# taichi-dev/voxel-rt2

Hardware: AMD Instinct MI355X
Metric: Mpath-samples/sec at 1920x1080, 8 bounces (higher is better)
Workload: dtype f32; 1 GPU; example1-style scene S1 (scenes.scene_s1), 128^3 grid, 1920x1080, 4 spp/step, 8 bounces, static camera, ReSTIR off; width=1920, height=1080, max_depth=8, seed=0, build_id=fbd5f3073040a2f2

## Files before the change

voxel_rt2_amd/csrc/vrt_kernels.hip:

```cpp
#include <hip/hip_runtime.h>
#include <cstdlib>
#include <atomic>
#include "vrt_kernels.h"
#include "vrt_probe.h"
#include "vrt_shade_probe.h"

namespace vrt {

template <int G>
__global__ void k_pack_grid(const int8_t* __restrict__ mat, const uint8_t* __restrict__ rgb, uint32_t* __restrict__ grid) {
    int i = blockIdx.x * blockDim.x + threadIdx.x;
    if (i >= G * G * G) return;
    int m = mat[i];
    uint32_t a = (m < 0) ? 0u : (uint32_t)m;
    const int z = i & (G - 1), y = (i / G) & (G - 1), x = i / (G * G);
    grid[texel_index<G>(x, y, z)] = (uint32_t)rgb[3 * i] | ((uint32_t)rgb[3 * i + 1] << 8) | ((uint32_t)rgb[3 * i + 2] << 16) | (a << 24);
}
__global__ void k_build_l0(const int8_t* __restrict__ mat, unsigned long long* __restrict__ l0, int G) {
    int b = blockIdx.x * blockDim.x + threadIdx.x;
    const int n0 = G >> 2;
    if (b >= n0 * n0 * n0) return;
    int bx = b % n0, by = (b / n0) % n0, bz = b / (n0 * n0);
    unsigned long long w = 0ULL;
    for (int z = 0; z < 4; z++)
// ... 355 lines not shown
    TraceStats ts;
    stats_zero(ts);
    bool exhausted = false;
    const unsigned tiles_per_range = ((unsigned)(tiles_x * tiles_y) + VRT_WORK_HEADS - 1u) / VRT_WORK_HEADS;
    const unsigned range = tiles_per_range * 64u * (unsigned)n_samples;
    const uint32_t prim_tag = drain_value;
    unsigned head = blockIdx.x & (VRT_WORK_HEADS - 1u);
    int heads_left = VRT_WORK_HEADS;
    unsigned q_cont = 0u, q_left = 0u;
    if constexpr (QUEUED) {
        q_cont = pq.counts[head * VRT_PV_COUNT_STRIDE]; q_left = pq.counts[head * VRT_PV_COUNT_STRIDE + 1];
        q_cont = q_cont < pq.cap ? q_cont : pq.cap; q_left = q_left < pq.left_cap ? q_left : pq.left_cap;
    }

#if defined(VRT_DIAG_REGIONS)
    unsigned long long t_prev = __builtin_readcyclecounter();
    int prev_stage = 4;
    unsigned long long t_stage[6] = {0ULL, 0ULL, 0ULL, 0ULL, 0ULL, 0ULL};
    unsigned long long t_sub[4] = {0ULL, 0ULL, 0ULL, 0ULL};
#define VRT_SUB_CLOCK(q) do { __asm__ volatile("s_waitcnt vmcnt(0) lgkmcnt(0)" ::: "memory"); const unsigned long long t_ = __builtin_readcyclecounter(); t_sub[q] += t_ - t_sub_prev; t_sub_prev = t_; } while (0)
#define VRT_SUB_START() do { __asm__ volatile("s_waitcnt vmcnt(0) lgkmcnt(0)" ::: "memory"); t_sub_prev = __builtin_readcyclecounter(); } while (0)
    unsigned long long t_sub_prev = 0ULL;
#define VRT_POOL_CLOCK(next_stage)                                                                              \
    do {                                                                                                        \
        const unsigned long long t_now = __builtin_readcyclecounter();                                          \
        _Pragma("unroll") for (int q_ = 0; q_ < 6; q_++) if (prev_stage == q_) t_stage[q_] += t_now - t_prev;   \
        t_prev = t_now; prev_stage = (next_stage);                                                              \
    } while (0)
#else
#define VRT_POOL_CLOCK(next_stage) ((void)0)
#define VRT_SUB_CLOCK(q) ((void)0)
#define VRT_SUB_START() ((void)0)
#endif
    for (;;) {
        wave_lds_sync();
        VRT_POOL_CLOCK(5);
        uint32_t st[WORDS];
        int cnt[4] = {0, 0, 0, 0};
#pragma unroll
        for (int k = 0; k < WORDS; k++) {
            st[k] = state[k * 64 + lane];
#pragma unroll
            for (int q = 0; q < 4; q++) cnt[q] += __popcll(__ballot(st[k] == (uint32_t)q));
        }
        if (exhausted) cnt[SLOT_EMPTY] = 0;
        int stage = SLOT_SHADE, best = cnt[SLOT_SHADE];
        if (cnt[SLOT_ESCAPE] > best) { stage = SLOT_ESCAPE; best = cnt[SLOT_ESCAPE]; }
        if (cnt[SLOT_RAY] > best) { stage = SLOT_RAY; best = cnt[SLOT_RAY]; }
        if (cnt[SLOT_EMPTY] > best) { stage = SLOT_EMPTY; best = cnt[SLOT_EMPTY]; }
        if (best == 0) break;
        int n = 0;
#pragma unroll
        for (int k = 0; k < WORDS; k++) {
            const bool mine = st[k] == (uint32_t)stage;
            const unsigned long long m = __ballot(mine);
            if (mine) list[n + lane_rank(m)] = (uint32_t)(k * 64 + lane);
            n += __popcll(m);
        }
        wave_lds_sync();
        VRT_POOL_CLOCK(stage);

        if (stage == SLOT_RAY) {
            VRT_REGION(14);
#ifndef VRT_POOL_PARK_MIN
#define VRT_POOL_PARK_MIN 64
#endif
            const int park = (n >= VRT_POOL_PARK_MIN) ? VRT_POOL_PARK : 0;
            int head = 0;
            bool active = false, ended = false;
            RayWalk w;
            BrickCache bc;
            bc.key = -1; bc.word = 0ULL;
            CoarseWords cw;
            cw.w1 = 0ULL; cw.w2 = 0ULL;
            SlotRef s;
            s.base = pool; s.stride = SLOTS;
            int slot = 0, iters0 = 0;
            for (;;) {
                const unsigned long long idle = __ballot(!active);
                const int n_idle = __popcll(idle);
                if (ended) {
                    VRT_REGION(16);
                    walk_store(s, w);
                    state[slot] = (uint32_t)slot_state_after_walk<G>(w.t, s.f(PF_FLOOR_T));
                    if (prim_cache) {
                        const uint32_t ids = s.u(PF_IDS);
                        if ((ids >> 24) == 0u)
                            primary_record_store(&prim_cache[((int)((ids >> 12) & 0xfffu) - fp.row0) * fp.W + (int)(ids & 0xfffu)], primary_record(s, prim_tag));
                    }
                    ts.iters += (unsigned)(w.iters - iters0);
                    ended = false;
                }
                if (head >= n) {
                    if (64 - n_idle <= park) {
                        if (active) {
                            VRT_REGION(17);
                            walk_store(s, w);
                            ts.iters += (unsigned)(w.iters - iters0);
                        }
                        break;
                    }
                } else {
                    const int idx = head + lane_rank(idle);
                    if (!active && idx < n) {
                        VRT_REGION(15);
                        slot = (int)list[idx];
                        s.base = pool + slot;
                        walk_load<G>(s, w);
                        coarse_fetch(P, w.ix, w.iy, w.iz, cw);
                        bc.key = -1;
                        iters0 = w.iters;
                        active = true;
                    }
                    head += (n_idle < n - head) ? n_idle : n - head;
                }
                const int target = (head < n) ? VRT_POOL_REFILL : 64 - park;
                do {
                    if (active) {
                        int nq;
                        if (walk_trip(P, w, bc, cw, nq)) { active = false; ended = true; }
                        ts.queries += (unsigned)nq;
                    }
                } while (__popcll(__ballot(!active)) < target);
            }
        } else {
            const int take = n < 64 ? n : 64;
            unsigned base = 0u, limit = 0u;
            unsigned range0 = 0u, per_sample = 1u;
            unsigned q_head = 0u, q_n_cont = 0u;
            if constexpr (QUEUED) {
              if (stage == SLOT_EMPTY) {
                VRT_SUB_START();
                unsigned got = 0u;
                if (lane == 0) got = atomicAdd(work_counter + head * VRT_WORK_HEAD_STRIDE, (unsigned)take);
                got = (unsigned)__builtin_amdgcn_readfirstlane((int)got);
                const unsigned cnt = q_cont + q_left;
                q_head = head; q_n_cont = q_cont;
                base = got;
                limit = (got + (unsigned)take < cnt) ? got + (unsigned)take : cnt;
                if (got + (unsigned)take >= cnt) {
                    heads_left -= 1;
                    head = (head + 1u) & (VRT_WORK_HEADS - 1u);
                    q_cont = pq.counts[head * VRT_PV_COUNT_STRIDE]; q_left = pq.counts[head * VRT_PV_COUNT_STRIDE + 1];
                    q_cont = q_cont < pq.cap ? q_cont : pq.cap; q_left = q_left < pq.left_cap ? q_left : pq.left_cap;
                    if (heads_left == 0) {
                        exhausted = true;
                        if (drain_signal && lane == 0 && atomicExch(work_counter + 1, 1u) == 0u)
                            __hip_atomic_fetch_max(drain_signal, drain_value, __ATOMIC_RELAXED, __HIP_MEMORY_SCOPE_SYSTEM);
                    }
                }
                if (base > limit) base = limit;
                VRT_SUB_CLOCK(0);
              }
            } else
            if (stage == SLOT_EMPTY) {
                VRT_SUB_START();
                unsigned got = 0u;
                if (lane == 0) got = atomicAdd(work_counter + head * VRT_WORK_HEAD_STRIDE, (unsigned)take);
                got = (unsigned)__builtin_amdgcn_readfirstlane((int)got);
                const unsigned r0 = head * range, r1 = (r0 + range < total) ? r0 + range : total;
                base = r0 + got;
                limit = (base + (unsigned)take < r1) ? base + (unsigned)take : r1;
                range0 = r0;
                per_sample = (r1 > r0) ? (r1 - r0) / (unsigned)n_samples : 1u;
                if (r0 >= total || base + (unsigned)take >= r1) {
                    heads_left -= 1;
                    head = (head + 1u) & (VRT_WORK_HEADS - 1u);
                    if (heads_left == 0) {
                        exhausted = true;
                        if (drain_signal && lane == 0 && atomicExch(work_counter + 1, 1u) == 0u)
                            __hip_atomic_fetch_max(drain_signal, drain_value, __ATOMIC_RELAXED, __HIP_MEMORY_SCOPE_SYSTEM);
                    }
                }
                if (base > limit) base = limit;
                VRT_SUB_CLOCK(0);
            }
            if (lane < take) {
                SlotRef s;
                s.stride = SLOTS;
                if (stage == SLOT_SHADE) {
                    VRT_REGION(11);
                    const int slot = (int)list[lane];
                    s.base = pool + slot;
                    state[slot] = (uint32_t)pool_shade<HIT_SOMETHING, BLACK_SUN, RESTIR>(fp, scl, P, out, s, cold_wave + slot * COLD, ts);
                } else if (stage == SLOT_ESCAPE) {
                    VRT_REGION(12);
                    const int slot = (int)list[lane];
                    s.base = pool + slot;
                    state[slot] = (uint32_t)pool_shade<HIT_NOTHING, false, RESTIR>(fp, scl, P, out, s, cold_wave + slot * COLD, ts);
                } else {
                    VRT_REGION(13);
                    const unsigned my = base + (unsigned)lane;
                    if constexpr (QUEUED) {
                        if (my < limit) {
                            const int slot = (int)list[lane];
                            s.base = pool + slot;
                            if (my < q_n_cont) {
                                constexpr int PW = PrimaryContWords<BLACK_SUN>::count;
                                const uint32_t* const at = pq.entries + ((size_t)q_head * pq.cap + my) * PW;
                                uint32_t e[PW];
#pragma unroll
                                for (int k = 0; k < PW; k++) e[k] = at[k];
                                VRT_SUB_CLOCK(1);
                                state[slot] = (uint32_t)pool_begin_queued<G, CULL, BLACK_SUN>(fp, scl.cull, s, cold_wave + slot * COLD, e, ts);
                                VRT_SUB_CLOCK(3);
                            } else {
                                const uint32_t item = pq.leftovers[(size_t)q_head * pq.left_cap + (my - q_n_cont)];
                                const int u = (int)(item & 0xfffu), v = (int)((item >> 12) & 0xfffu), sample = (int)(item >> 28);
                                const PrimaryRecord rec = primary_record_load(&prim_cache[(v - fp.row0) * fp.W + u]);
                                const bool known = primary_record_valid(rec, prim_tag);
                                VRT_SUB_CLOCK(1);
                                int st;
                                if (known) st = pool_begin_known<G>(fp, s, u, v, sample, rec);
                                else {
                                    st = pool_begin<G, CULL>(fp, scl.cull, s, u, v, sample, ts);
                                    if (sample == 0 && st != SLOT_RAY) primary_record_store(&prim_cache[(v - fp.row0) * fp.W + u], primary_record(s, prim_tag));
                                }
                                state[slot] = (uint32_t)st;
                                VRT_SUB_CLOCK(known ? 2 : 3);
                            }
                        }
                    } else
                    if (my < limit) {
                        const int slot = (int)list[lane];
                        s.base = pool + slot;
                        const unsigned j = my - range0;
                        const int sample = (int)(j >= per_sample) + (int)(j >= 2u * per_sample) + (int)(j >= 3u * per_sample);
                        const unsigned rem = j - (unsigned)sample * per_sample;
                        const unsigned tile = range0 / (64u * (unsigned)n_samples) + (rem >> 6), in = rem & 63u;
                        const int u = (int)(tile % (unsigned)tiles_x) * 8 + (int)(in & 7u);
                        const int v = launch_tile_row(fp, (int)(tile / (unsigned)tiles_x)) + (int)(in >> 3);
                        if (u < fp.W && v < fp.row1 && launch_renders_row(fp, v) && !outside_render_area(fp, (float)u, (float)v)) {
                            bool known = false;
                            PrimaryRecord rec;
                            rec.x = rec.y = rec.z = rec.dx = rec.dy = rec.dz = rec.ft = rec.w = 0u;
                            if (prim_cache && (SERVED || sample > 0)) {
                                rec = primary_record_load(&prim_cache[(v - fp.row0) * fp.W + u]);
                                known = primary_record_valid(rec, prim_tag);
                            }
                            VRT_SUB_CLOCK(1);
                            int st;
                            if (known) st = pool_begin_known<G>(fp, s, u, v, sample, rec);
                            else {
                                st = pool_begin<G, CULL>(fp, scl.cull, s, u, v, sample, ts);
                                if (prim_cache && sample == 0 && st != SLOT_RAY) primary_record_store(&prim_cache[(v - fp.row0) * fp.W + u], primary_record(s, prim_tag));
                            }
                            state[slot] = (uint32_t)st;
                            VRT_SUB_CLOCK(known ? 2 : 3);
                        }
                    }
                }
            }
        }
    }
    VRT_POOL_CLOCK(4);
#if defined(VRT_DIAG_REGIONS)
    if (lane == 0)
        for (int q = 0; q < 6; q++) atomicAdd(&g_vrt_region[2 * (20 + q)], t_stage[q]);
    if (lane == 0)
        for (int q = 0; q < 4; q++) atomicAdd(&g_vrt_region[52 + q], t_sub[q]);
#endif
    if (INSTR) flush_stats(ts, sc.counters);
}
template <int G, bool INSTR, bool BLACK_SUN, bool CULL, bool SERVED = false>
__global__ __launch_bounds__(64 * pool_shape<G>(false).waves, VRT_POOL_MIN_WAVES) __attribute__((amdgpu_num_vgpr(VRT_POOL_HALF_VGPRS))) void k_render_pool(FrameParams fp, SceneData sc, PixelBuffers out, unsigned* work_counter, unsigned* next_counter, int n_samples, uint32_t* cold, uint32_t* drain_signal, uint32_t drain_value, PrimaryRecord* prim_cache) {
    render_pool_body<G, false, INSTR, BLACK_SUN, CULL, false, SERVED>(fp, sc, out, work_counter, next_counter, n_samples, cold, drain_signal, drain_value, prim_cache);
}
template <int G, bool INSTR, bool CULL>
__global__ __launch_bounds__(64 * pool_shape<G>(true).waves, 3) __attribute__((amdgpu_num_vgpr(84))) void k_render_pool_dense12(FrameParams fp, SceneData sc, PixelBuffers out, unsigned* work_counter, unsigned* next_counter, int n_samples, uint32_t* cold, uint32_t* drain_signal, uint32_t drain_value, PrimaryRecord* prim_cache) {
    render_pool_body<G, false, INSTR, false, CULL, true>(fp, sc, out, work_counter, next_counter, n_samples, cold, drain_signal, drain_value, prim_cache);
}
template <int G, bool INSTR, bool CULL>
__global__ __launch_bounds__(64 * pool_shape<G>(false).waves, VRT_POOL_MIN_WAVES) __attribute__((amdgpu_num_vgpr(128))) void k_render_pool_restir(FrameParams fp, SceneData sc, PixelBuffers out, unsigned* work_counter, unsigned* next_counter, int n_samples, uint32_t* cold, uint32_t* drain_signal, uint32_t drain_value, PrimaryRecord* prim_cache) {
    render_pool_body<G, true, INSTR, false, CULL>(fp, sc, out, work_counter, next_counter, n_samples, cold, drain_signal, drain_value, prim_cache);
}

#ifndef VRT_PRIMARY_HALF_VGPRS
#define VRT_PRIMARY_HALF_VGPRS 48
#endif
template <int G, bool CULL>
__global__ __launch_bounds__(64) __attribute__((amdgpu_num_vgpr(VRT_PRIMARY_HALF_VGPRS))) void k_primary_records(FrameParams fp, SceneData sc, PrimaryRecord* prim_cache, uint32_t tag) {
    const int tiles_x = (fp.W + 7) >> 3;
    const unsigned tile = blockIdx.x, in = threadIdx.x;
    const int u = (int)(tile % (unsigned)tiles_x) * 8 + (int)(in & 7u);
    const int v = launch_tile_row(fp, (int)(tile / (unsigned)tiles_x)) + (int)(in >> 3);
    if (!(u < fp.W && v < fp.row1 && launch_renders_row(fp, v) && !outside_render_area(fp, (float)u, (float)v))) return;
    GlobalPyramid<G> P;
    P.p = sc.pyr;
    primary_record_store(&prim_cache[(v - fp.row0) * fp.W + u], primary_record_walk<G, CULL>(fp, P, sc.cull, u, v, tag));
}

#ifndef VRT_PRIMARY_VERTEX_HALF_VGPRS
#define VRT_PRIMARY_VERTEX_HALF_VGPRS 72
#endif
#ifndef VRT_PRIMARY_VERTEX_SUN_HALF_VGPRS
#define VRT_PRIMARY_VERTEX_SUN_HALF_VGPRS 84
#endif
#if 2 * VRT_PRIMARY_VERTEX_HALF_VGPRS + 2 * VRT_POOL_HALF_VGPRS > 512 || 2 * VRT_PRIMARY_VERTEX_SUN_HALF_VGPRS + 2 * VRT_POOL_HALF_VGPRS > 512
#error "k_primary_vertex must fit beside one pooled wave of a SIMD at least"
#endif
#ifndef VRT_PRIMARY_SHARED_SURF
#define VRT_PRIMARY_SHARED_SURF 1
#endif
template <int G, bool BLACK_SUN, bool CULL>
static __device__ __forceinline__ void primary_vertex_body(const FrameParams& fp, const SceneData& sc, const PixelBuffers& out, const PrimaryRecord* prim_cache, uint32_t tag, int n_samples, const PrimaryQueue& pq) {
    const int tiles_x = (fp.W + 7) >> 3;
    const unsigned tile = blockIdx.x, in = threadIdx.x;
    const int u = (int)(tile % (unsigned)tiles_x) * 8 + (int)(in & 7u);
    const int v = launch_tile_row(fp, (int)(tile / (unsigned)tiles_x)) + (int)(in >> 3);
    const bool live = u < fp.W && v < fp.row1 && launch_renders_row(fp, v) && !outside_render_area(fp, (float)u, (float)v);
    const unsigned head = tile & (VRT_PV_HEADS - 1u);
    constexpr int PW = PrimaryContWords<BLACK_SUN>::count;
    GlobalPyramid<G> P;
    P.p = sc.pyr;
    TraceStats ts;
    stats_zero(ts);
    PrimaryRecord rec;
    rec.x = rec.y = rec.z = rec.dx = rec.dy = rec.dz = rec.ft = rec.w = 0u;
    bool known = false;
    Hit h;
    hit_init(h);
    int state = SLOT_ESCAPE;
    constexpr bool SHARED_SURF = VRT_PRIMARY_SHARED_SURF != 0;
    Surf surf;
#if defined(VRT_DIAG_REGIONS)
    __shared__ unsigned long long pv_clock[PVR_COUNT + 1];
    if (in <= (unsigned)PVR_COUNT) pv_clock[in] = 0ULL;
    ts.pv = pv_clock;
    ts.pv[PVR_COUNT] = __builtin_readcyclecounter();
#endif
    if (live) {
        rec = primary_record_load(&prim_cache[(v - fp.row0) * fp.W + u]);
        known = primary_record_valid(rec, tag);
    }
    VRT_PV_CLOCK(ts, PVR_RECORD);
    if (known) {
        state = primary_vertex_hit<G>(fp, sc, rec, h, ts);
        primary_vertex_gbuffer(fp, out, u, v, rec, h);
        VRT_PV_CLOCK(ts, PVR_HIT);
        if constexpr (SHARED_SURF) (void)primary_vertex_surf<GlobalPyramid<G>>(sc, rec, h, state, surf);
        VRT_PV_CLOCK(ts, PVR_SURF);
    }
    unsigned n_done = 0u, n_on = 0u;
    for (int sample = 0; sample < n_samples; sample++) {
        Path<false> p;
        bool on = false;
        if (known) on = primary_vertex_sample<G, BLACK_SUN, CULL, SHARED_SURF>(fp, sc, P, out, u, v, sample, rec, h, state, p, ts, &surf);
        const unsigned long long m_on = __ballot(on);
        bool left = live && !known;
        if (m_on != 0ULL) {
            unsigned at = 0u;
            if (in == (unsigned)__builtin_ctzll(m_on)) at = atomicAdd(&pq.counts[head * VRT_PV_COUNT_STRIDE], (unsigned)__popcll(m_on));
            at = (unsigned)__shfl((int)at, __builtin_ctzll(m_on), 64) + (unsigned)__popcll(m_on & ((1ULL << in) - 1ULL));
            if (on) {
                if (at < pq.cap) primary_cont_pack<BLACK_SUN>(pq.entries + ((size_t)head * pq.cap + at) * PW, p);
                else left = true;
            }
        }
        const unsigned long long m_left = __ballot(left);
        if (m_left != 0ULL) {
            unsigned at = 0u;
            if (in == (unsigned)__builtin_ctzll(m_left)) at = atomicAdd(&pq.counts[head * VRT_PV_COUNT_STRIDE + 1], (unsigned)__popcll(m_left));
            at = (unsigned)__shfl((int)at, __builtin_ctzll(m_left), 64) + (unsigned)__popcll(m_left & ((1ULL << in) - 1ULL));
            if (left && at < pq.left_cap) pq.leftovers[(size_t)head * pq.left_cap + at] = primary_leftover_item(u, v, sample);
        }
        if (known && !left) { if (on) n_on++; else n_done++; }
        VRT_PV_CLOCK(ts, PVR_APPEND);
    }
#if defined(VRT_DIAG_REGIONS)
    if (in < (unsigned)PVR_COUNT) atomicAdd(&g_vrt_region[56 + in], pv_clock[in]);
    static_assert(56 + PVR_COUNT <= 64, "the region counters' last eight words");
#endif
    if (pq.report) {
        unsigned long long a = n_done, b = n_on;
        for (int off = 32; off > 0; off >>= 1) { a += __shfl_down(a, off, 64); b += __shfl_down(b, off, 64); }
        if (in == 0u) { atomicAdd(&pq.report[0], a); atomicAdd(&pq.report[1], b); }
    }
}
template <int G, bool CULL>
__global__ __launch_bounds__(64) __attribute__((amdgpu_num_vgpr(VRT_PRIMARY_VERTEX_HALF_VGPRS))) void k_primary_vertex(FrameParams fp, SceneData sc, PixelBuffers out, const PrimaryRecord* prim_cache, uint32_t tag, int n_samples, PrimaryQueue pq) {
    primary_vertex_body<G, true, CULL>(fp, sc, out, prim_cache, tag, n_samples, pq);
}
template <int G, bool CULL>
__global__ __launch_bounds__(64) __attribute__((amdgpu_num_vgpr(VRT_PRIMARY_VERTEX_SUN_HALF_VGPRS))) void k_primary_vertex_sun(FrameParams fp, SceneData sc, PixelBuffers out, const PrimaryRecord* prim_cache, uint32_t tag, int n_samples, PrimaryQueue pq) {
    primary_vertex_body<G, false, CULL>(fp, sc, out, prim_cache, tag, n_samples, pq);
}
template <int G, bool BLACK_SUN, bool CULL>
__global__ __launch_bounds__(64 * pool_shape<G>(false).waves, VRT_POOL_MIN_WAVES) __attribute__((amdgpu_num_vgpr(VRT_POOL_HALF_VGPRS))) void k_render_pool_queued(FrameParams fp, SceneData sc, PixelBuffers out, unsigned* work_counter, unsigned* next_counter, int n_samples, uint32_t* cold, uint32_t* drain_signal, uint32_t drain_value, PrimaryRecord* prim_cache, PrimaryQueue pq) {
    render_pool_body<G, false, false, BLACK_SUN, CULL, false, true, true>(fp, sc, out, work_counter, next_counter, n_samples, cold, drain_signal, drain_value, prim_cache, pq);
}

#ifndef VRT_GRIS_SPLIT
#define VRT_GRIS_SPLIT 1
#endif
#ifndef VRT_GRIS_MIN_WAVES
#define VRT_GRIS_MIN_WAVES 2
#endif
#ifndef VRT_GRIS_MIN_WAVES_A
#define VRT_GRIS_MIN_WAVES_A 3
#endif
#ifndef VRT_GRIS_MIN_WAVES_B
#define VRT_GRIS_MIN_WAVES_B 3
#endif
template <int G, bool INSTR, int PHASE = 0>
__global__ __launch_bounds__(256, (PHASE == 1 ? VRT_GRIS_MIN_WAVES_A : PHASE == 2 ? VRT_GRIS_MIN_WAVES_B : VRT_GRIS_MIN_WAVES)) void k_gris(FrameParams fp, SceneData sc, GrisBuffers gb, int r0, int r_first, int r1, int tiles_x, int band_w) {
    constexpr int N1 = GridDim<G>::n1 * GridDim<G>::n1 * GridDim<G>::n1, N2 = GridDim<G>::n2 * GridDim<G>::n2 * GridDim<G>::n2;
    __shared__ unsigned long long s_l1[N1];
    __shared__ unsigned long long s_l2[N2];
    __shared__ float s_mats[128 * 14];
    __shared__ float s_mats_x[128 * 8];
    __shared__ float s_cs[4][64];
    __shared__ uint16_t s_off[32][256];
    for (int i = threadIdx.x; i < N1; i += blockDim.x) s_l1[i] = sc.pyr.l1[i];
    if (threadIdx.x < N2) s_l2[threadIdx.x] = sc.pyr.l2[threadIdx.x];
    for (int i = threadIdx.x; i < 128 * 14; i += blockDim.x) s_mats[i] = sc.mats[i];
    for (int i = threadIdx.x; i < 128 * 8; i += blockDim.x) s_mats_x[i] = gb.mats_x[i];
    __shared__ float s_cull[8];
    if (threadIdx.x < 8) s_cull[threadIdx.x] = sc.cull[threadIdx.x];
    LdsPyramid<G, INSTR> P;
    P.l0 = sc.pyr.l0; P.l1 = s_l1; P.l2 = s_l2;
    P.w3 = (G == 256) ? sc.pyr.l3[0] : 0ULL;
    P.oob = sc.pyr.ref_oob != 0;
    SceneData scl = sc;
    scl.mats = s_mats;
    scl.cull = s_cull;
    GrisBuffers gbl = gb;
    gbl.mats_x = s_mats_x;
    const int xcd = blockIdx.x & 7, slot = blockIdx.x >> 3;
    const int bx = xcd * band_w + slot % band_w, by = slot / band_w;
    const int wave = threadIdx.x >> 6, lane = threadIdx.x & 63;
    const int u = bx * 16 + (wave & 1) * 8 + (lane & 7);
    const int v = r0 + by * 16 + (wave >> 1) * 8 + (lane >> 3);
    if (lane < 32) gris_tap_cs(u, v, 0, lane, s_cs[wave]);
    __syncthreads();
    GrisTaps taps;
    taps.cs = s_cs[wave]; taps.off = &s_off[0][threadIdx.x]; taps.off_stride = 256;
    TraceStats ts;
    stats_zero(ts);
    if (bx < tiles_x && u < fp.W && v >= r_first && v < r1) gris_pixel<PHASE>(fp, scl, P, gbl, taps, u, v, 0, 24.0f, 32, 1, ts);
    if (INSTR) flush_stats(ts, sc.counters);
}

#ifndef VRT_GRIS_FIRST_ROUNDS
#define VRT_GRIS_FIRST_ROUNDS 1
#endif
template <int G, bool INSTR>
__global__ __launch_bounds__(256, VRT_GRIS_MIN_WAVES_A) void k_gris_first(FrameParams fp, SceneData sc, GrisBuffers gb, int r0, int r_first, int r1, int tiles_x, int band_w) {
    __shared__ float s_mats[128 * 14];
    __shared__ float s_mats_x[128 * 8];
    __shared__ float s_cs[4][64];
    __shared__ uint32_t s_item[4][64 * 32 / VRT_GRIS_FIRST_ROUNDS];
    __shared__ float s_radius[4][64];
    for (int i = threadIdx.x; i < 128 * 14; i += blockDim.x) s_mats[i] = sc.mats[i];
    for (int i = threadIdx.x; i < 128 * 8; i += blockDim.x) s_mats_x[i] = gb.mats_x[i];
    SceneData scl = sc;
    scl.mats = s_mats;
    GrisBuffers gbl = gb;
    gbl.mats_x = s_mats_x;
    const int xcd = blockIdx.x & 7, slot = blockIdx.x >> 3;
    const int bx = xcd * band_w + slot % band_w, by = slot / band_w;
    const int wave = threadIdx.x >> 6, lane = threadIdx.x & 63;
    const int u0 = bx * 16 + (wave & 1) * 8, v0 = r0 + by * 16 + (wave >> 1) * 8;
    const int u = u0 + (lane & 7), v = v0 + (lane >> 3);
    if (lane < 32) gris_tap_cs(u, v, 0, lane, s_cs[wave]);
    __syncthreads();
    GrisTaps taps;
    taps.cs = s_cs[wave]; taps.off = nullptr; taps.off_stride = 0;
    TraceStats ts;
    stats_zero(ts);
    const int max_taps = 32;
    const float max_radius = 24.0f;
    uint32_t* const item = s_item[wave];

    const int idx = (v - fp.row0) * fp.W + u;
    bool mine = bx < tiles_x && u < fp.W && v >= r_first && v < r1 && !outside_render_area(fp, (float)u, (float)v);
    unsigned accepted = 0u, walk = 0u;
    float const_term = 0.0f;
    if (mine) {
        const GrisGeo* cg = &gb.geo[idx];
        if (near_zero3(cg->x1)) mine = false;
        else {
            dm_rng rng = dm_rng_init(fp.seed, fp.frame, (uint32_t)(v * fp.W + u), 1u);
            (void)dm_rng_f32(&rng);
            s_radius[wave][lane] = dm_rng_f32(&rng);
            accepted = cg->pad;
            walk = accepted & gb.src[idx].pad2;
            Reservoir c;
            c.z.F = gb.src[idx].F; c.M = gb.src[idx].M;
            const_term = gris_first_const_term(c, max_taps);
        }
    }
    float canonical_mis = 1.0f;
    constexpr int ROUNDS = VRT_GRIS_FIRST_ROUNDS, PER = 64 / ROUNDS;
    for (int round = 0; round < ROUNDS; round++) {
        const bool in_round = lane / PER == round;
        const int cnt = in_round ? __builtin_popcount(walk) : 0;
        int incl = cnt;
        for (int off = 1; off < 64; off <<= 1) {
            const int up = __shfl_up(incl, off, 64);
            if (lane >= off) incl += up;
        }
        const int base = incl - cnt;
        const int total = __shfl(incl, 63, 64);
        if (in_round) {
            int k = base;
            for (unsigned m = walk; m != 0u; m &= m - 1u) item[k++] = ((uint32_t)lane << 8) | (uint32_t)__builtin_ctz(m);
        }
        wave_lds_sync();
        for (int k0 = 0; k0 < total; k0 += 64) {
            const int k = k0 + lane;
            if (k < total) {
                const uint32_t e = item[k];
                const int q = (int)(e >> 8), i = (int)(e & 31u);
                const int uq = u0 + (q & 7), vq = v0 + (q >> 3);
                int tx, ty;
                (void)gris_tap(fp, taps, uq, vq, i, s_radius[wave][q], max_radius, max_taps, tx, ty);
                Reservoir center;
                f3 center_rc_ty, center_sky_t;
                RcPre center_pre;
                gris_load_src(center, center_rc_ty, center_sky_t, center_pre, gb.src[(vq - fp.row0) * fp.W + uq]);
                item[k] = dm_f2u(gris_first_term(fp, scl, gbl, center, center_rc_ty, center_sky_t, center_pre, tx, ty, max_taps, ts));
            }
        }
        wave_lds_sync();
        if (mine && in_round) {
            int k = base;
            for (unsigned m = accepted; m != 0u; m &= m - 1u) {
                const int i = __builtin_ctz(m);
                canonical_mis += ((walk >> i) & 1u) ? dm_u2f(item[k++]) : const_term;
            }
            gb.geo[idx].pad3 = dm_f2u(canonical_mis);
        }
        wave_lds_sync();
    }
    if (INSTR) flush_stats(ts, sc.counters);
}

#ifndef VRT_CLASSIFY_MIN_WAVES
#define VRT_CLASSIFY_MIN_WAVES 4
#endif
template <bool INSTR>
__global__ __launch_bounds__(256, VRT_CLASSIFY_MIN_WAVES) void k_gris_classify(FrameParams fp, SceneData sc, GrisBuffers gb, int r0, int r_first, int r1, int tiles_x, int band_w) {
    __shared__ float s_cs[4][64];
    const int xcd = blockIdx.x & 7, slot = blockIdx.x >> 3;
    const int bx = xcd * band_w + slot % band_w, by = slot / band_w;
    const int wave = threadIdx.x >> 6, lane = threadIdx.x & 63;
    const int u = bx * 16 + (wave & 1) * 8 + (lane & 7);
    const int v = r0 + by * 16 + (wave >> 1) * 8 + (lane >> 3);
    if (lane < 32) gris_tap_cs(u, v, 0, lane, s_cs[wave]);
    __syncthreads();
    GrisTaps taps;
    taps.cs = s_cs[wave]; taps.off = nullptr; taps.off_stride = 0;
    TraceStats ts;
    stats_zero(ts);
    if (bx < tiles_x && u < fp.W && v >= r_first && v < r1) gris_classify_pixel(fp, gb, taps, u, v, 24.0f, 32, ts);
    if (INSTR) flush_stats(ts, sc.counters);
}

__global__ __launch_bounds__(256) void k_gris_prepare(FrameParams fp, SceneData sc, GrisBuffers gb) {
    const int u = blockIdx.x * 64 + (threadIdx.x & 63);
    const int v = fp.row0 + blockIdx.y * 4 + (threadIdx.x >> 6);
    if (u < fp.W && v < fp.row1) gris_prepare_pixel(fp, sc, gb, u, v);
}
__global__ void k_mat_derived(const float* mats, float* mats_x) {
    const int id = threadIdx.x;
    if (id < 128) { const Material m = load_material(mats, id); store_mat_derived(mats_x, id, mat_derive(m), material_unit_range(m)); }
}

#ifndef VRT_TEMPORAL_HALF_VGPRS
#define VRT_TEMPORAL_HALF_VGPRS 48
#endif
#ifndef VRT_TEMPORAL_ROWS
#define VRT_TEMPORAL_ROWS 1
#endif
__global__ __launch_bounds__(64 * VRT_TEMPORAL_ROWS) __attribute__((amdgpu_num_vgpr(VRT_TEMPORAL_HALF_VGPRS))) void k_temporal(FrameParams fp, TemporalBuffers tb, int r0, int r1, int n_samples) {
    const int u = blockIdx.x * 64 + (threadIdx.x & 63);
    const int v = r0 + blockIdx.y * VRT_TEMPORAL_ROWS + (threadIdx.x >> 6);
    if (u < fp.W && v < r1) temporal_pixel(fp, tb, u, v, n_samples);
}
__global__ __launch_bounds__(64 * VRT_TEMPORAL_ROWS) __attribute__((amdgpu_num_vgpr(VRT_TEMPORAL_HALF_VGPRS))) void k_temporal_stripes(FrameParams fp, TemporalBuffers tb, int n_own, int n_samples) {
    const int u = blockIdx.x * 64 + (threadIdx.x & 63);
    const int k = blockIdx.y * VRT_TEMPORAL_ROWS + (threadIdx.x >> 6);
    if (k >= n_own) return;
    const int v = (k / fp.stripe_rows) * fp.stripe_period + fp.stripe_first + k % fp.stripe_rows;
    if (u < fp.W && v < fp.H) temporal_pixel<true>(fp, tb, u, v, n_samples);
}
__global__ __launch_bounds__(64 * VRT_TEMPORAL_ROWS) __attribute__((amdgpu_num_vgpr(VRT_TEMPORAL_HALF_VGPRS))) void k_temporal_frame_prev(FrameParams fp, TemporalBuffers tb, int r0, int r1, int n_samples) {
    const int u = blockIdx.x * 64 + (threadIdx.x & 63);
    const int v = r0 + blockIdx.y * VRT_TEMPORAL_ROWS + (threadIdx.x >> 6);
    if (u < fp.W && v < r1) temporal_pixel<false, true>(fp, tb, u, v, n_samples);
}
__global__ __launch_bounds__(64 * VRT_TEMPORAL_ROWS) __attribute__((amdgpu_num_vgpr(VRT_TEMPORAL_HALF_VGPRS))) void k_temporal_group(TemporalGroup tg, int r0, int r1) {
    const int u = blockIdx.x * 64 + (threadIdx.x & 63);
    const int v = r0 + blockIdx.y * VRT_TEMPORAL_ROWS + (threadIdx.x >> 6);
    if (u < tg.W && v < r1) temporal_group_pixel(tg, u, v);
}
__global__ __launch_bounds__(256) void k_tonemap(FrameParams fp, const f3* hdr, f4* ldr, int r0, int r1) {
    const int u = blockIdx.x * 64 + (threadIdx.x & 63);
    const int v = r0 + blockIdx.y * 4 + (threadIdx.x >> 6);
    if (u < fp.W && v < r1) ldr[(v - fp.row0) * fp.W + u] = tonemap_pixel(fp, hdr, u, v);
}
__global__ __launch_bounds__(256) void k_tonemap8(FrameParams fp, const f3* hdr, uint32_t* ldr8, int r0, int r1) {
    const int u = blockIdx.x * 64 + (threadIdx.x & 63);
    const int v = r0 + blockIdx.y * 4 + (threadIdx.x >> 6);
    if (u < fp.W && v < r1) {
        const f4 c = tonemap_pixel(fp, hdr, u, v);
        ldr8[(v - fp.row0) * fp.W + u] = dm_f2u32(dm_saturate(c.x) * 255.0f + 0.5f) | (dm_f2u32(dm_saturate(c.y) * 255.0f + 0.5f) << 8) |
                                         (dm_f2u32(dm_saturate(c.z) * 255.0f + 0.5f) << 16) | (dm_f2u32(dm_saturate(c.w) * 255.0f + 0.5f) << 24);
    }
}
__global__ __launch_bounds__(256) void k_denoise_prepare(int W, int H, int moving, DenoiseSource src, DenoiseGuide* __restrict__ guide, uint32_t* __restrict__ mat,
                                                         f4* __restrict__ d, f4* __restrict__ s, f3* __restrict__ out) {
    const int u = blockIdx.x * 64 + (threadIdx.x & 63);
    const int v = blockIdx.y * 4 + (threadIdx.x >> 6);
    if (u >= W || v >= H) return;
    const int idx = v * W + u;
    const uint32_t M = src.gb_mat[idx];
    DenoiseGuide g;
    f4 xd, xs;
    const bool surface = denoise_prepare(src.gb_pos[idx], src.gb_normal[idx], M, src.hist_d[idx], src.hist_s[idx], moving, g, xd, xs);
    guide[idx] = g;
    mat[idx] = M;
    d[idx] = xd;
    s[idx] = xs;
    if (!surface) out[idx] = src.hdr[idx];
}
template <int S>
__global__ __launch_bounds__(256) void k_denoise_atrous(DenoiseIn in, DenoiseSettings st, int use_lum, f4* __restrict__ d_out, f4* __restrict__ s_out,
                                                        const f4* __restrict__ u_d, const f4* __restrict__ u_s, f3* __restrict__ out) {
    const int u = blockIdx.x * 32 + (threadIdx.x & 31);
    const int v = blockIdx.y * 8 + (threadIdx.x >> 5);
    if (u >= in.W || v >= in.H) return;
    const int idx = v * in.W + u;
    f4 xd, xs;
    const bool surface = denoise_iteration(in, u, v, S, use_lum != 0, st.sigma_l, st.tol, xd, xs);
    if (out) {
        if (surface) out[idx] = denoise_finish(xd, xs, u_d[idx], u_s[idx], in.mat[idx], st.moving, st.full_at);
    } else {
        d_out[idx] = xd;
        s_out[idx] = xs;
    }
}
#if defined(VRT_DIAG_REGIONS)
__global__ void k_diag_read(unsigned long long* out, int reset) {
    int i = threadIdx.x;
    if (i < 64) { out[i] = g_vrt_region[i]; if (reset) g_vrt_region[i] = 0ULL; }
}
#endif
hipError_t launch_diag_read(hipStream_t st, unsigned long long* out, int reset) {
#if defined(VRT_DIAG_REGIONS)
    hipLaunchKernelGGL(k_diag_read, dim3(1), dim3(64), 0, st, out, reset);
    return hipGetLastError();
#else
    (void)st; (void)out; (void)reset;
    return hipErrorNotSupported;
#endif
}
__global__ void k_detmath_probe(int op, int n, const float* a, const float* b, float* out) {
    int i = blockIdx.x * blockDim.x + threadIdx.x;
    if (i >= n) return;
    float r = 0.0f;
    switch (op) {
        case 0: r = dm_sin(a[i]); break;
        case 1: r = dm_cos(a[i]); break;
        case 2: r = dm_exp(a[i]); break;
        case 3: r = dm_log(a[i]); break;
        case 4: r = dm_pow(a[i], b[i]); break;
        case 5: r = dm_acos(a[i]); break;
// ... 1027 lines not shown
```

voxel_rt2_amd/csrc/vrt_primary.h:

```cpp
#ifndef VRT_PRIMARY_H
#define VRT_PRIMARY_H

#include "vrt_pool.h"

namespace vrt {

enum {
    PV_POS = 0, PV_DIR = 3, PV_THR = 6, PV_RNG = 9,
    PV_IDS = 10,
    PV_INVPDF = 11, PV_MAT = 12, PV_PPOS = 13,
    PV_COUNT = 16,
    PV_NEE_D = 16, PV_NEE_S = 19, PV_COUNT_SUN = 24
};
template <bool BLACK_SUN> struct PrimaryContWords { static constexpr int count = BLACK_SUN ? (int)PV_COUNT : (int)PV_COUNT_SUN; };
#define VRT_PV_COUNT_STRIDE 32

struct PrimaryQueue {
    uint32_t* counts;
    uint32_t* entries;
    uint32_t* leftovers;
    uint32_t cap, left_cap;
    unsigned long long* report;
};
#define VRT_PV_HEADS 8

VRT_DEV uint32_t primary_leftover_item(int u, int v, int sample) { return (uint32_t)u | ((uint32_t)v << 12) | ((uint32_t)sample << 28); }

template <int G>
VRT_DEV int primary_vertex_hit(const FrameParams& fp, const SceneData& sc, const PrimaryRecord& rec, Hit& h, TraceStats& ts) {
    hit_init(h);
    const int state = slot_state_after_walk<G>(dm_u2f(rec.x), dm_u2f(rec.ft));
    if (state == SLOT_SHADE) {
        const f3 d = mk3(dm_u2f(rec.dx), dm_u2f(rec.dy), dm_u2f(rec.dz));
        const float ft = dm_u2f(rec.ft);
        if (ft < DM_INF) hit_floor(fp, d, ft, h);
        const uint32_t a = rec.y, b = rec.z;
        TraceOut tr;
        walk_result(d, dm_u2f(rec.x), (int)(int16_t)(a & 0xffffu), (int)(int16_t)(a >> 16), (int)(int16_t)(b & 0xffffu), normal_decode(b >> 20), 0, tr);
        hit_voxel<false, G>(fp, sc, world_to_voxel<G>(fp.camera_pos), d, tr, h, ts);
    }
    return state;
}

VRT_DEV void primary_vertex_gbuffer(const FrameParams& fp, const PixelBuffers& out, int u, int v, const PrimaryRecord& rec, const Hit& h) {
    const int local_idx = (v - fp.row0) * fp.W + u;
    const f3 hit_pos = fp.camera_pos + h.closest * mk3(dm_u2f(rec.dx), dm_u2f(rec.dy), dm_u2f(rec.dz));
    const f3 ppos = (h.closest == DM_INF) ? mk3(0.0f) : hit_pos;
    stream_store(&out.gb_normal[local_idx], oct_encode(h.normal));
    stream_store3(&out.gb_position[local_idx], ppos);
    stream_store(&out.gb_mat[local_idx], pack_material(h.mat_id, h.albedo));
    stream_store(&out.gb_depth[local_idx], view_to_screen(xform(fp.view, ppos, 1.0f), fp.proj).z);
}

template <class PyrT>
VRT_DEV bool primary_vertex_surf(const SceneData& sc, const PrimaryRecord& rec, const Hit& h, int state, Surf& s) {
    if (!(state == SLOT_SHADE && !h.hit_light && h.closest < DM_INF)) return false;
    path_surf<PyrT>(sc, h, mk3(dm_u2f(rec.dx), dm_u2f(rec.dy), dm_u2f(rec.dz)), s);
    return true;
}

template <int G, bool BLACK_SUN, bool CULL, bool SHARED_SURF = false, class PyrT>
VRT_DEV bool primary_vertex_sample(const FrameParams& fp, const SceneData& sc, const PyrT& P, const PixelBuffers& out, int u, int v, int sample,
                                   const PrimaryRecord& rec, const Hit& h, int state, Path<false>& p, TraceStats& ts, const Surf* surf = nullptr) {
    path_begin_along(fp, p, u, v, sample, mk3(dm_u2f(rec.dx), dm_u2f(rec.dy), dm_u2f(rec.dz)));
    const int local_idx = (v - fp.row0) * fp.W + u;
    VRT_PV_CLOCK(ts, PVR_BEGIN);
    bool done;
    if (state == SLOT_SHADE) {
        done = path_shade<false, HIT_SOMETHING, BLACK_SUN, false, true, SHARED_SURF>(fp, sc, P, out, local_idx, p, h, ts, surf);
        VRT_PV_CLOCK(ts, PVR_SAMPLE);
    } else done = path_shade<false, HIT_NOTHING, false, false>(fp, sc, P, out, local_idx, p, h, ts);
    if (!done) {
        const float ft = floor_probe(fp, p.pos, p.d);
        RayWalk w;
        const bool alive = walk_prepare<G, CULL>(world_to_voxel<G>(p.pos), p.d, w, sc.cull);
        VRT_PV_CLOCK(ts, PVR_BOUNCE_RAY);
        if (alive || slot_state_after_walk<G>(w.t, ft) != SLOT_ESCAPE) return true;
        Hit none;
        hit_init(none);
        (void)path_shade<false, HIT_NOTHING, false>(fp, sc, P, out, local_idx, p, none, ts);
    }
    path_finish<false>(fp, sc, out, local_idx, p, ts);
    VRT_PV_CLOCK(ts, PVR_FINISH);
    return false;
}

template <bool BLACK_SUN>
VRT_DEV void primary_cont_pack(uint32_t* e, const Path<false>& p) {
    e[PV_POS] = dm_f2u(p.pos.x); e[PV_POS + 1] = dm_f2u(p.pos.y); e[PV_POS + 2] = dm_f2u(p.pos.z);
    e[PV_DIR] = dm_f2u(p.d.x); e[PV_DIR + 1] = dm_f2u(p.d.y); e[PV_DIR + 2] = dm_f2u(p.d.z);
    e[PV_THR] = dm_f2u(p.thr.x); e[PV_THR + 1] = dm_f2u(p.thr.y); e[PV_THR + 2] = dm_f2u(p.thr.z);
    e[PV_RNG] = p.rng.s;
    e[PV_IDS] = pack_ids(p.pix_u, p.pix_v, p.first_lobe, p.sample);
    e[PV_INVPDF] = dm_f2u(p.first_invpdf);
    e[PV_MAT] = p.primary_mat_info;
    e[PV_PPOS] = dm_f2u(p.primary_pos.x); e[PV_PPOS + 1] = dm_f2u(p.primary_pos.y); e[PV_PPOS + 2] = dm_f2u(p.primary_pos.z);
    if constexpr (!BLACK_SUN) {
        e[PV_NEE_D] = dm_f2u(p.nee_d.x); e[PV_NEE_D + 1] = dm_f2u(p.nee_d.y); e[PV_NEE_D + 2] = dm_f2u(p.nee_d.z);
        e[PV_NEE_S] = dm_f2u(p.nee_s.x); e[PV_NEE_S + 1] = dm_f2u(p.nee_s.y); e[PV_NEE_S + 2] = dm_f2u(p.nee_s.z);
        e[PV_NEE_S + 3] = 0u; e[PV_NEE_S + 4] = 0u;
        static_assert(PV_NEE_S + 5 == PV_COUNT_SUN, "the record's padding");
    }
}
template <int G, bool CULL, bool BLACK_SUN>
VRT_DEV int pool_begin_queued(const FrameParams& fp, const float* cull, const SlotRef& s, uint32_t* cold_line, const uint32_t* e, TraceStats& ts) {
    Path<false> p;
    p.pos = mk3(dm_u2f(e[PV_POS]), dm_u2f(e[PV_POS + 1]), dm_u2f(e[PV_POS + 2]));
    p.d = mk3(dm_u2f(e[PV_DIR]), dm_u2f(e[PV_DIR + 1]), dm_u2f(e[PV_DIR + 2]));
    p.thr = mk3(dm_u2f(e[PV_THR]), dm_u2f(e[PV_THR + 1]), dm_u2f(e[PV_THR + 2]));
    p.contrib = mk3(0.0f);
    p.rng.s = e[PV_RNG];
    const uint32_t ids = e[PV_IDS];
    p.pix_u = (int)(ids & 0xfffu); p.pix_v = (int)((ids >> 12) & 0xfffu);
    p.depth = 1; p.sample = (int)(ids >> 28);
    p.first_lobe = (int)((ids >> 24) & 15u); p.sky_primary = 0;
    p.refl_dist = 0.0f;
    p.first_invpdf = dm_u2f(e[PV_INVPDF]);
    p.primary_mat_info = e[PV_MAT];
    p.primary_pos = mk3(dm_u2f(e[PV_PPOS]), dm_u2f(e[PV_PPOS + 1]), dm_u2f(e[PV_PPOS + 2]));
    p.primary_albedo = mk3(1.0f);
    if constexpr (BLACK_SUN) { p.nee_d = mk3(0.0f); p.nee_s = mk3(0.0f); }
    else {
        p.nee_d = mk3(dm_u2f(e[PV_NEE_D]), dm_u2f(e[PV_NEE_D + 1]), dm_u2f(e[PV_NEE_D + 2]));
        p.nee_s = mk3(dm_u2f(e[PV_NEE_S]), dm_u2f(e[PV_NEE_S + 1]), dm_u2f(e[PV_NEE_S + 2]));
    }
    path_store_cold(cold_line, p);
    path_store_hot(s, p);
    return pool_launch_ray<G, CULL>(fp, cull, s, p.pos, p.d, ts);
}

}
#endif
```

Measured before the change: 12750 Mpath-samples/s.

## Split primary vertex into head/tail, hoist queue atomic, shade plain escapes once

Splits the per-sample primary vertex into a head (shade plus bounce-ray setup) and a tail (escape shading and finish). The continuation-queue atomic is now issued before the tail of non-continuing lanes, so its latency overlaps that work. Waves whose known lanes all escape to a non-sky background shade the escape once and only repeat path_finish per sample. Risks: the escape-once path assumes the escape shading does not depend on the sample index or RNG, and the added inline-asm barriers may change register allocation.

Measured after the change: 12640 Mpath-samples/s. About the same (-0.8%).

```diff
diff --git a/voxel_rt2_amd/csrc/vrt_kernels.hip b/voxel_rt2_amd/csrc/vrt_kernels.hip
--- a/voxel_rt2_amd/csrc/vrt_kernels.hip
+++ b/voxel_rt2_amd/csrc/vrt_kernels.hip
@@ -681,6 +681,20 @@
 #ifndef VRT_PRIMARY_SHARED_SURF
 #define VRT_PRIMARY_SHARED_SURF 1
 #endif
+#ifndef VRT_PRIMARY_EARLY_ATOMIC
+#define VRT_PRIMARY_EARLY_ATOMIC 1
+#endif
+#ifndef VRT_PRIMARY_ESCAPE_ONCE
+#define VRT_PRIMARY_ESCAPE_ONCE 1
+#endif
+static __device__ __forceinline__ void primary_leftover_append(const PrimaryQueue& pq, unsigned head, unsigned in, bool left, int u, int v, int sample) {
+    const unsigned long long m_left = __ballot(left);
+    if (m_left == 0ULL) return;
+    unsigned at = 0u;
+    if (in == (unsigned)__builtin_ctzll(m_left)) at = atomicAdd(&pq.counts[head * VRT_PV_COUNT_STRIDE + 1], (unsigned)__popcll(m_left));
+    at = (unsigned)__shfl((int)at, __builtin_ctzll(m_left), 64) + (unsigned)__popcll(m_left & ((1ULL << in) - 1ULL));
+    if (left && at < pq.left_cap) pq.leftovers[(size_t)head * pq.left_cap + at] = primary_leftover_item(u, v, sample);
+}
 template <int G, bool BLACK_SUN, bool CULL>
 static __device__ __forceinline__ void primary_vertex_body(const FrameParams& fp, const SceneData& sc, const PixelBuffers& out, const PrimaryRecord* prim_cache, uint32_t tag, int n_samples, const PrimaryQueue& pq) {
     const int tiles_x = (fp.W + 7) >> 3;
@@ -721,28 +735,51 @@
         VRT_PV_CLOCK(ts, PVR_SURF);
     }
     unsigned n_done = 0u, n_on = 0u;
+#if VRT_PRIMARY_ESCAPE_ONCE
+    const bool plain = primary_escapes_plain(fp, known, state);
+    if (__ballot(plain) != 0ULL && __ballot(known && !plain) == 0ULL) {
+        Path<false> p;
+        if (plain) primary_escape_once(fp, sc, P, out, u, v, rec, h, p, ts);
+        for (int sample = 0; sample < n_samples; sample++) {
+            if (plain) primary_escape_sample(fp, sc, out, u, v, sample, p, ts);
+            primary_leftover_append(pq, head, in, live && !known, u, v, sample);
+            VRT_PV_CLOCK(ts, PVR_APPEND);
+        }
+        if (plain) n_done += (unsigned)n_samples;
+        n_samples = 0;
+    }
+#endif
     for (int sample = 0; sample < n_samples; sample++) {
         Path<false> p;
-        bool on = false;
-        if (known) on = primary_vertex_sample<G, BLACK_SUN, CULL, SHARED_SURF>(fp, sc, P, out, u, v, sample, rec, h, state, p, ts, &surf);
+        int outcome = PV_ENDS;
+        if (known) outcome = primary_vertex_head<G, BLACK_SUN, CULL, SHARED_SURF>(fp, sc, P, out, u, v, sample, rec, h, state, p, ts, &surf);
+        const bool on = known && outcome == PV_GOES_ON;
         const unsigned long long m_on = __ballot(on);
+        unsigned at = 0u;
+#if VRT_PRIMARY_EARLY_ATOMIC
+        if (m_on != 0ULL && in == (unsigned)__builtin_ctzll(m_on)) {
+            unsigned zero;
+            __asm__ volatile("v_mov_b32 %0, 0" : "=v"(zero));
+            at = atomicAdd(&pq.counts[head * VRT_PV_COUNT_STRIDE] + zero, (unsigned)__popcll(m_on));
+        }
+#endif
+        if (known && !on) {
+            int tu = u, tv = v;
+            __asm__ volatile("" : "+v"(tu), "+v"(tv));
+            primary_vertex_tail(fp, sc, P, out, tu, tv, outcome, p, ts);
+        }
         bool left = live && !known;
         if (m_on != 0ULL) {
-            unsigned at = 0u;
+#if !VRT_PRIMARY_EARLY_ATOMIC
             if (in == (unsigned)__builtin_ctzll(m_on)) at = atomicAdd(&pq.counts[head * VRT_PV_COUNT_STRIDE], (unsigned)__popcll(m_on));
+#endif
             at = (unsigned)__shfl((int)at, __builtin_ctzll(m_on), 64) + (unsigned)__popcll(m_on & ((1ULL << in) - 1ULL));
             if (on) {
                 if (at < pq.cap) primary_cont_pack<BLACK_SUN>(pq.entries + ((size_t)head * pq.cap + at) * PW, p);
                 else left = true;
             }
         }
-        const unsigned long long m_left = __ballot(left);
-        if (m_left != 0ULL) {
-            unsigned at = 0u;
-            if (in == (unsigned)__builtin_ctzll(m_left)) at = atomicAdd(&pq.counts[head * VRT_PV_COUNT_STRIDE + 1], (unsigned)__popcll(m_left));
-            at = (unsigned)__shfl((int)at, __builtin_ctzll(m_left), 64) + (unsigned)__popcll(m_left & ((1ULL << in) - 1ULL));
-            if (left && at < pq.left_cap) pq.leftovers[(size_t)head * pq.left_cap + at] = primary_leftover_item(u, v, sample);
-        }
+        primary_leftover_append(pq, head, in, left, u, v, sample);
         if (known && !left) { if (on) n_on++; else n_done++; }
         VRT_PV_CLOCK(ts, PVR_APPEND);
     }
diff --git a/voxel_rt2_amd/csrc/vrt_primary.h b/voxel_rt2_amd/csrc/vrt_primary.h
--- a/voxel_rt2_amd/csrc/vrt_primary.h
+++ b/voxel_rt2_amd/csrc/vrt_primary.h
@@ -59,9 +59,10 @@
     return true;
 }
 
+enum { PV_GOES_ON = 0, PV_ESCAPES = 1, PV_ENDS = 2 };
 template <int G, bool BLACK_SUN, bool CULL, bool SHARED_SURF = false, class PyrT>
-VRT_DEV bool primary_vertex_sample(const FrameParams& fp, const SceneData& sc, const PyrT& P, const PixelBuffers& out, int u, int v, int sample,
-                                   const PrimaryRecord& rec, const Hit& h, int state, Path<false>& p, TraceStats& ts, const Surf* surf = nullptr) {
+VRT_DEV int primary_vertex_head(const FrameParams& fp, const SceneData& sc, const PyrT& P, const PixelBuffers& out, int u, int v, int sample,
+                                const PrimaryRecord& rec, const Hit& h, int state, Path<false>& p, TraceStats& ts, const Surf* surf = nullptr) {
     path_begin_along(fp, p, u, v, sample, mk3(dm_u2f(rec.dx), dm_u2f(rec.dy), dm_u2f(rec.dz)));
     const int local_idx = (v - fp.row0) * fp.W + u;
     VRT_PV_CLOCK(ts, PVR_BEGIN);
@@ -70,19 +71,46 @@
         done = path_shade<false, HIT_SOMETHING, BLACK_SUN, false, true, SHARED_SURF>(fp, sc, P, out, local_idx, p, h, ts, surf);
         VRT_PV_CLOCK(ts, PVR_SAMPLE);
     } else done = path_shade<false, HIT_NOTHING, false, false>(fp, sc, P, out, local_idx, p, h, ts);
-    if (!done) {
-        const float ft = floor_probe(fp, p.pos, p.d);
-        RayWalk w;
-        const bool alive = walk_prepare<G, CULL>(world_to_voxel<G>(p.pos), p.d, w, sc.cull);
-        VRT_PV_CLOCK(ts, PVR_BOUNCE_RAY);
-        if (alive || slot_state_after_walk<G>(w.t, ft) != SLOT_ESCAPE) return true;
+    if (done) return PV_ENDS;
+    const float ft = floor_probe(fp, p.pos, p.d);
+    RayWalk w;
+    const bool alive = walk_prepare<G, CULL>(world_to_voxel<G>(p.pos), p.d, w, sc.cull);
+    VRT_PV_CLOCK(ts, PVR_BOUNCE_RAY);
+    return (alive || slot_state_after_walk<G>(w.t, ft) != SLOT_ESCAPE) ? PV_GOES_ON : PV_ESCAPES;
+}
+template <class PyrT>
+VRT_DEV void primary_vertex_tail(const FrameParams& fp, const SceneData& sc, const PyrT& P, const PixelBuffers& out, int u, int v, int outcome,
+                                 Path<false>& p, TraceStats& ts) {
+    const int local_idx = (v - fp.row0) * fp.W + u;
+    if (outcome == PV_ESCAPES) {
         Hit none;
         hit_init(none);
         (void)path_shade<false, HIT_NOTHING, false>(fp, sc, P, out, local_idx, p, none, ts);
     }
     path_finish<false>(fp, sc, out, local_idx, p, ts);
     VRT_PV_CLOCK(ts, PVR_FINISH);
+}
+template <int G, bool BLACK_SUN, bool CULL, bool SHARED_SURF = false, class PyrT>
+VRT_DEV bool primary_vertex_sample(const FrameParams& fp, const SceneData& sc, const PyrT& P, const PixelBuffers& out, int u, int v, int sample,
+                                   const PrimaryRecord& rec, const Hit& h, int state, Path<false>& p, TraceStats& ts, const Surf* surf = nullptr) {
+    const int outcome = primary_vertex_head<G, BLACK_SUN, CULL, SHARED_SURF>(fp, sc, P, out, u, v, sample, rec, h, state, p, ts, surf);
+    if (outcome == PV_GOES_ON) return true;
+    primary_vertex_tail(fp, sc, P, out, u, v, outcome, p, ts);
     return false;
+}
+
+VRT_DEV bool primary_escapes_plain(const FrameParams& fp, bool known, int state) { return known && state == SLOT_ESCAPE && fp.use_sky != 1; }
+template <class PyrT>
+VRT_DEV void primary_escape_once(const FrameParams& fp, const SceneData& sc, const PyrT& P, const PixelBuffers& out, int u, int v,
+                                 const PrimaryRecord& rec, const Hit& h, Path<false>& p, TraceStats& ts) {
+    path_begin_along(fp, p, u, v, 0, mk3(dm_u2f(rec.dx), dm_u2f(rec.dy), dm_u2f(rec.dz)));
+    VRT_PV_CLOCK(ts, PVR_BEGIN);
+    (void)path_shade<false, HIT_NOTHING, false, false>(fp, sc, P, out, (v - fp.row0) * fp.W + u, p, h, ts);
+}
+VRT_DEV void primary_escape_sample(const FrameParams& fp, const SceneData& sc, const PixelBuffers& out, int u, int v, int sample, Path<false>& p, TraceStats& ts) {
+    p.sample = sample;
+    path_finish<false>(fp, sc, out, (v - fp.row0) * fp.W + u, p, ts);
+    VRT_PV_CLOCK(ts, PVR_FINISH);
 }
 
 template <bool BLACK_SUN>
```
